# PaiDii/TGTC-Style

Hardware: AMD Instinct MI355X
Metric: rays/sec (128c+64f samples) on fern 400x400 (higher is better)
Workload: dtype f16 MFMA product + two block-scaled fp6 (e2m3) correction products, f32 accumulate (fine pass; coarse pass: fp16x3); 1 GPU; fern-shaped 400x400 frame, plain NeRF render (style off), 128 coarse + 64 fine samples/ray, one whole frame per rank per step, seeded random-init weights; precision=fp16x3+fp16mx

## Files before the change

tgtc-style_amd/csrc/mlp_nerf_fp16s.hip:

```cpp
#define TGTC_ASM_DMA 1
#include "mlp_nerf_mx.h"

#include <cstdlib>

#include "mlp_layouts.h"

namespace tgtc {

#ifndef TGTC_FP16S_INC
#define TGTC_FP16S_INC "fp16s_asm_nerf.inc"
#endif
#include TGTC_FP16S_INC

using CfgFp16s = MlpCfg<4, kFp16sTiles, false, 4>;
#ifndef TGTC_FRONT_ABL
#define TGTC_FRONT_ABL 0
#endif

__device__ __forceinline__ unsigned udiv_word(unsigned n) {
    unsigned z = (unsigned)(__builtin_amdgcn_rcpf((float)n) * 4294966784.0f);
    return z + __umulhi(z, (0u - n) * z);
}

template <int IN_MODE, int NCT>
__device__ __forceinline__ void fp16s_front(const NerfArgs& a, long long s_wave, half8 (&keep)[NCT][2], unsigned& bad) {
    const int lane = fresh_lane_id();
    const int g = lane >> 4, n = lane & 15;
    double pos[NCT][3], dir[NCT][3];
    long long sidx[NCT];
    half8 pe_h[2][NCT], pe_l[2][NCT], de_h[1][NCT], de_l[1][NCT];
    bad = 0;
#if TGTC_FRONT_ABL & 1
#pragma unroll
    for (int c = 0; c < NCT; ++c) pe_h[0][c] = pe_h[1][c] = half8{(_Float16)(float)(g + n)};
#else
    nerf_load_samples<NCT, IN_MODE>(a, s_wave, n, pos, dir, sidx);
    nerf_encode<NCT, false, false>(a, pos, dir, sidx, g, pe_h, pe_l, de_h, de_l);
#pragma unroll
    for (int c = 0; c < NCT; ++c)
        if (!(__builtin_fabs(pos[c][0]) <= kScreenBox && __builtin_fabs(pos[c][1]) <= kScreenBox && __builtin_fabs(pos[c][2]) <= kScreenBox))
            bad |= 1u << c;
#endif
#pragma unroll
    for (int c = 0; c < NCT; ++c) keep[c][0] = pe_h[0][c], keep[c][1] = pe_h[1][c];
}

template <int IN_MODE, bool FRONT>
__global__ void __launch_bounds__(256, 1) nerf_fp16s_kernel(NerfArgs a, long long n_pass) {
    using C = CfgFp16s;
    constexpr int NCT = C::NCT;
    using Ring = WeightStream<C, SingleStreamMap<NerfLayout::kFragsSigma>, true, true>;
    constexpr int kChunk = kFp16sChunkBytes, kSlots = C::RING_BYTES / kChunk, kLook = kSlots - 1, kPiece = kChunk / C::NWAVES;
    constexpr int kPad = ((NerfLayout::kFragsSigma * C::FRAG_BYTES + kChunk - 1) / kChunk + kSlots - 1) / kSlots * kSlots;
    static_assert(NerfLayout::kFragsSigma == kFp16sFrags && kPad == kFp16sPadChunks && C::RING_BYTES == 131072 && C::FRAG_BYTES == 1024 &&
                      kPiece % 4096 == 0 && kChunk == kChunkBytes,
                  "the generated stream was laid out for this ring");
    static_assert(kFp16sBox == kScreenBox, "the generated front end tests positions against the HIP front end's box");
    static_assert(!FRONT || IN_MODE == IN_RAYS, "the in-stream front end loads samples of rays");

    __shared__ __attribute__((aligned(16))) char smem[C::RING_BYTES + kNerfBiasBytes];
    const int wave = __builtin_amdgcn_readfirstlane(threadIdx.x >> 6);
    Ring ring;
    {
        const int lane = threadIdx.x & 63;
        const char* const streams[1] = {a.stream};
        ring.init(streams, smem, wave, lane);
#pragma unroll
        for (int j = 0; j < kNerfBiasBytes / (C::NWAVES * 1024); ++j)
            lds_dma16(a.bias + (j * C::NWAVES + wave) * 1024 + lane * 16, smem + C::RING_BYTES + (j * C::NWAVES + wave) * 1024);
        ring.lds_wave = smem + wave * kPiece;
        ring.voff = wave * kPiece + lane * 16;
        static_for<kLook * (kPiece / 1024)>([&](auto i_) {
            constexpr int i = decltype(i_)::value, ch = i / (kPiece / 1024), j = i % (kPiece / 1024);
            lds_dma16_s<(j % 4) * 1024>(ring.src[0] + ch * kChunk + (j / 4) * 4096, ring.voff, ring.lds_wave + ch * kChunk + (j / 4) * 4096);
        });
    }

    unsigned bad = 0;
    half8 keep[NCT][2];
    if constexpr (FRONT) {
        fp16s_front<IN_MODE>(a, (long long)blockIdx.x * C::SAMPLES_PER_WG + wave * C::SAMPLES_PER_WAVE, keep, bad);
        fp16s_asm_first_keep(keep);
    }
    const unsigned mm1 = (unsigned)(a.M - 1), zz = __builtin_amdgcn_readfirstlane(udiv_word((unsigned)a.N));

    for (long long p = blockIdx.x; p < n_pass; p += gridDim.x) {
        const long long s_wave = p * C::SAMPLES_PER_WG + wave * C::SAMPLES_PER_WAVE;
        if constexpr (!FRONT) fp16s_front<IN_MODE>(a, s_wave, keep, bad);
        const int fl = fresh_lane_id();
        ring.voff = wave * kPiece + fl * 16;
        ring.lane_lo = opaque((lds_cptr)smem + fl * 16);
        ring.lane_hi = opaque((lds_cptr)smem + 65536 + fl * 16);
        const lds_cptr bias_lane = opaque((lds_cptr)smem + C::RING_BYTES + 16 * (fl >> 4));
        float sigma[NCT];
        unsigned nbad = 0;
        if constexpr (FRONT) {
            const unsigned snext = (unsigned)(s_wave + (long long)gridDim.x * C::SAMPLES_PER_WG);
            fp16s_asm_nerf_sigma_pass_front(ring, bias_lane, sigma, nbad, a.ts, a.rays_o, a.rays_d, mm1, (unsigned)a.N, zz, snext);
        } else {
            fp16s_asm_nerf_sigma_pass(ring, bias_lane, keep, sigma);
        }
        const int lane = fresh_lane_id();
        if (lane < 16) {
#pragma unroll
            for (int c = 0; c < NCT; ++c) {
                const long long s = s_wave + c * 16 + lane;
                if (s < a.M) a.sigma[s] = (bad >> c & 1) ? __builtin_nanf("") : sigma[c];
            }
        }
        if constexpr (FRONT) bad = nbad;
    }
    wait_vmcnt<0>();
}

int nerf_fp16s_launch(const NerfArgs& a, hipStream_t st) {
    using C = CfgFp16s;
    if (a.M <= 0) return TGTC_OK;
    if (a.M >= 0x7fffffffLL) return fail(TGTC_ERR_UNSUPPORTED, "nerf: too many samples in one launch (%lld)", a.M);
    int cus = 0;
    if (const int rc = cu_count(cus)) return rc;
    const long long n_pass = (a.M + C::SAMPLES_PER_WG - 1) / C::SAMPLES_PER_WG;
    const unsigned grid = (unsigned)(n_pass < cus ? n_pass : cus);
    const char* e = std::getenv("TGTC_SCREEN_SERIAL_FRONT");
    if (e && e[0] == '1') nerf_fp16s_kernel<IN_RAYS, false><<<grid, C::NWAVES * 64, 0, st>>>(a, n_pass);
    else nerf_fp16s_kernel<IN_RAYS, true><<<grid, C::NWAVES * 64, 0, st>>>(a, n_pass);
    TGTC_LAUNCH_CHECK();
    return TGTC_OK;
}

}
```

tgtc-style_amd/csrc/mlp_nerf_front.h:

```cpp
#pragma once
#include "mlp_core.h"

namespace tgtc {

enum InMode { IN_RAYS = 0, IN_PTS = 1, IN_ENC = 2, IN_LIST = 3 };

struct NerfArgs {
    const char* bias;
    const char* stream;
    long long M;
    int N;
    const double* rays_o;
    const double* rays_d;
    const float* ts;
    const double* pts;
    const double* dirs;
    const float* pts_enc;
    const float* dirs_enc;
    float* rgb;
    float* sigma;
    float* remap;
    float* out_pts_enc;
    float* out_dirs_enc;
    const unsigned* live;
    const unsigned* n_live;
};

template <int NCT, int IN_MODE>
__device__ __forceinline__ void nerf_load_samples(const NerfArgs& a, long long s_wave, int n, double (&pos)[NCT][3],
                                                  double (&dir)[NCT][3], long long (&sidx)[NCT], unsigned n_live = 0) {
#pragma unroll
    for (int c = 0; c < NCT; ++c) {
        long long s = s_wave + c * 16 + n;
        if constexpr (IN_MODE == IN_LIST) {
            const unsigned i = (unsigned long long)s < n_live ? (unsigned)s : n_live - 1;
            s = a.live[i];
        }
        sidx[c] = s;
        if (s >= a.M) s = a.M - 1;
        if constexpr (IN_MODE == IN_RAYS || IN_MODE == IN_LIST) {
            const long long r = (unsigned)s / (unsigned)a.N;
            const double t = (double)a.ts[s];
#pragma unroll
            for (int k = 0; k < 3; ++k) {
                dir[c][k] = a.rays_d[r * 3 + k];
                pos[c][k] = a.rays_o[r * 3 + k] + t * dir[c][k];
            }
        } else if constexpr (IN_MODE == IN_PTS) {
#pragma unroll
            for (int k = 0; k < 3; ++k) pos[c][k] = a.pts[s * 3 + k], dir[c][k] = a.dirs[s * 3 + k];
        }
        if constexpr (IN_MODE != IN_ENC) {
#pragma unroll
            for (int k = 0; k < 3; ++k) asm volatile("" : "+v"(pos[c][k]), "+v"(dir[c][k]));
        }
    }
}

template <int NCT, bool SPLIT, bool FULL>
__device__ __forceinline__ void nerf_load_encoded(const NerfArgs& a, const long long (&sidx)[NCT], int g,
                                                  half8 (&pe_h)[2][NCT], half8 (&pe_l)[2][NCT], half8 (&de_h)[1][NCT],
                                                  half8 (&de_l)[1][NCT]) {
#pragma unroll
    for (int c = 0; c < NCT; ++c) {
        const long long s = sidx[c] < a.M ? sidx[c] : a.M - 1;
        half8 h2[2], l2[2];
        load_encoded_point<SPLIT>(a.pts_enc + s * 63, g, h2, l2);
        pe_h[0][c] = h2[0], pe_h[1][c] = h2[1], pe_l[0][c] = l2[0], pe_l[1][c] = l2[1];
        if constexpr (FULL) load_encoded_dir<SPLIT>(a.dirs_enc + s * 27, g, de_h[0][c], de_l[0][c]);
    }
}

template <int NCT, bool SPLIT, bool FULL>
__device__ __forceinline__ void nerf_encode(const NerfArgs& a, const double (&pos)[NCT][3], const double (&dir)[NCT][3],
                                            const long long (&sidx)[NCT], int g, half8 (&pe_h)[2][NCT],
                                            half8 (&pe_l)[2][NCT], half8 (&de_h)[1][NCT], half8 (&de_l)[1][NCT]) {
#pragma unroll
    for (int c = 0; c < NCT; ++c) {
        const bool live = sidx[c] < a.M;
        half8 h2[2], l2[2];
        encode_point<SPLIT, SPLIT>(pos[c], g, h2, l2, (a.out_pts_enc && live) ? a.out_pts_enc + sidx[c] * 63 : nullptr);
        pe_h[0][c] = h2[0], pe_h[1][c] = h2[1], pe_l[0][c] = l2[0], pe_l[1][c] = l2[1];
        if constexpr (FULL) {
            bool same = false;
            if constexpr (NCT > 1) {
                if (c > 0 && !a.out_dirs_enc)
                    same = __all(dir[c][0] == dir[c - 1][0] && dir[c][1] == dir[c - 1][1] && dir[c][2] == dir[c - 1][2]);
            }
            if (same) {
                de_h[0][c] = de_h[0][c > 0 ? c - 1 : 0], de_l[0][c] = de_l[0][c > 0 ? c - 1 : 0];
            } else {
                encode_dir<SPLIT, SPLIT>(dir[c], g, de_h[0][c], de_l[0][c],
                                         (a.out_dirs_enc && live) ? a.out_dirs_enc + sidx[c] * 27 : nullptr);
            }
        }
    }
}

template <int IN_MODE, bool SPLIT>
__device__ __forceinline__ void nerf_encode_dir_late(const NerfArgs& a, long long sidx, int g, half8& de_h, half8& de_l) {
    const long long s = sidx < a.M ? sidx : a.M - 1;
    if constexpr (IN_MODE == IN_ENC) {
        load_encoded_dir<SPLIT>(a.dirs_enc + s * 27, g, de_h, de_l);
    } else {
        double d[3];
        const double* src = (IN_MODE == IN_RAYS || IN_MODE == IN_LIST) ? a.rays_d + ((unsigned)s / (unsigned)a.N) * 3 : a.dirs + s * 3;
#pragma unroll
        for (int k = 0; k < 3; ++k) d[k] = src[k];
        encode_dir<SPLIT, SPLIT>(d, g, de_h, de_l, (a.out_dirs_enc && sidx < a.M) ? a.out_dirs_enc + sidx * 27 : nullptr);
    }
}

}
```

tgtc-style_amd/csrc/mlp_nerf_x3s.hip:

```cpp
#define TGTC_ASM_DMA 1
#include "mlp_nerf_mx.h"

#include "mlp_layouts.h"

namespace tgtc {

#ifndef TGTC_X3S_INC
#define TGTC_X3S_INC "x3_asm_nerf.inc"
#endif
#include TGTC_X3S_INC

using CfgX3s = MlpCfg<4, 2, true, 4>;
#ifndef TGTC_FRONT_ABL
#define TGTC_FRONT_ABL 0
#endif

template <int IN_MODE>
__global__ void __launch_bounds__(256, 1) nerf_x3s_kernel(NerfArgs a, long long n_pass) {
    using C = CfgX3s;
    unsigned n_live = 0;
    if constexpr (IN_MODE == IN_LIST) {
        n_live = __builtin_amdgcn_readfirstlane(*a.n_live);
        n_pass = ((long long)n_live + C::SAMPLES_PER_WG - 1) / C::SAMPLES_PER_WG;
    }
    using Ring = WeightStream<C, SingleStreamMap<NerfLayout::kFragsSigma>, true, true>;
    constexpr int kChunk = kX3sChunkBytes, kSlots = C::RING_BYTES / kChunk, kLook = kSlots - 1, kPiece = kChunk / C::NWAVES;
    constexpr int kPad = ((NerfLayout::kFragsSigma * C::FRAG_BYTES + kChunk - 1) / kChunk + kSlots - 1) / kSlots * kSlots;
    static_assert(NerfLayout::kFragsSigma == kX3sFrags && kPad == kX3sPadChunks && C::RING_BYTES == 131072 && C::FRAG_BYTES == 2048 && kPiece % 4096 == 0,
                  "the generated stream was laid out for this ring");

    __shared__ __attribute__((aligned(16))) char smem[C::RING_BYTES + kNerfBiasBytes];
    const int wave = __builtin_amdgcn_readfirstlane(threadIdx.x >> 6);
    Ring ring;
    {
        const int lane = threadIdx.x & 63;
        const char* const streams[1] = {a.stream};
        ring.init(streams, smem, wave, lane);
#pragma unroll
        for (int j = 0; j < kNerfBiasBytes / (C::NWAVES * 1024); ++j)
            lds_dma16(a.bias + (j * C::NWAVES + wave) * 1024 + lane * 16, smem + C::RING_BYTES + (j * C::NWAVES + wave) * 1024);
        ring.lds_wave = smem + wave * kPiece;
        ring.voff = wave * kPiece + lane * 16;
        static_for<kLook * (kPiece / 1024)>([&](auto i_) {
            constexpr int i = decltype(i_)::value, ch = i / (kPiece / 1024), j = i % (kPiece / 1024);
            lds_dma16_s<(j % 4) * 1024>(ring.src[0] + ch * kChunk + (j / 4) * 4096, ring.voff, ring.lds_wave + ch * kChunk + (j / 4) * 4096);
        });
    }

    for (long long p = blockIdx.x; p < n_pass; p += gridDim.x) {
        const long long s_wave = p * C::SAMPLES_PER_WG + wave * C::SAMPLES_PER_WAVE;
        half8 keep[2][4];
        {
            const int lane = fresh_lane_id();
            const int g = lane >> 4, n = lane & 15;
            double pos[2][3], dir[2][3];
            long long sidx[2];
            half8 pe_h[2][2], pe_l[2][2], de_h[1][2], de_l[1][2];
#if TGTC_FRONT_ABL & 1
#pragma unroll
            for (int c = 0; c < 2; ++c) pe_h[0][c] = pe_h[1][c] = pe_l[0][c] = pe_l[1][c] = half8{(_Float16)(float)(g + n)};
#elif TGTC_FRONT_ABL & 4
            nerf_load_samples<2, IN_RAYS>(a, s_wave, n, pos, dir, sidx);
#pragma unroll
            for (int c = 0; c < 2; ++c)
                pe_h[0][c] = pe_h[1][c] = pe_l[0][c] = pe_l[1][c] = half8{(_Float16)(float)(pos[c][0] + pos[c][1] + pos[c][2])};
#else
            if constexpr (IN_MODE == IN_LIST) nerf_load_samples<2, IN_LIST>(a, s_wave, n, pos, dir, sidx, n_live);
            else nerf_load_samples<2, IN_RAYS>(a, s_wave, n, pos, dir, sidx);
            nerf_encode<2, true, false>(a, pos, dir, sidx, g, pe_h, pe_l, de_h, de_l);
#endif
#pragma unroll
            for (int c = 0; c < 2; ++c) keep[c][0] = pe_h[0][c], keep[c][1] = pe_h[1][c], keep[c][2] = pe_l[0][c], keep[c][3] = pe_l[1][c];
        }
        const int fl = fresh_lane_id();
        ring.voff = wave * kPiece + fl * 16;
        ring.lane_lo = opaque((lds_cptr)smem + fl * 16);
        ring.lane_hi = opaque((lds_cptr)smem + 65536 + fl * 16);
        const lds_cptr bias_lane = opaque((lds_cptr)smem + C::RING_BYTES + 16 * (fl >> 4));
        float sigma[2];
        x3_asm_nerf_sigma_pass(ring, wave, bias_lane, keep, sigma);
        const int lane = fresh_lane_id();
        if (lane < 16) {
#pragma unroll
            for (int c = 0; c < 2; ++c) {
                if constexpr (IN_MODE == IN_LIST) {
                    const unsigned long long slot = (unsigned long long)(s_wave + c * 16 + lane);
                    if (slot < n_live) {
                        const unsigned s = a.live[slot];
                        if (s < a.M) a.sigma[s] = sigma[c];
                    }
                    continue;
                }
                const long long s = s_wave + c * 16 + lane;
                if (s < a.M) a.sigma[s] = sigma[c];
            }
        }
    }
    wait_vmcnt<0>();
}

int nerf_x3s_launch(const NerfArgs& a, hipStream_t st) {
    using C = CfgX3s;
    int cus = 0;
    if (const int rc = cu_count(cus)) return rc;
    const long long n_pass = (a.M + C::SAMPLES_PER_WG - 1) / C::SAMPLES_PER_WG;
    nerf_x3s_kernel<IN_RAYS><<<(unsigned)(n_pass < cus ? n_pass : cus), C::NWAVES * 64, 0, st>>>(a, n_pass);
    TGTC_LAUNCH_CHECK();
    return TGTC_OK;
}

int nerf_x3s_list_launch(const NerfArgs& a, hipStream_t st) {
    using C = CfgX3s;
    int cus = 0;
    if (const int rc = cu_count(cus)) return rc;
    const long long n_pass = (a.M + C::SAMPLES_PER_WG - 1) / C::SAMPLES_PER_WG;
    nerf_x3s_kernel<IN_LIST><<<(unsigned)(n_pass < cus ? n_pass : cus), C::NWAVES * 64, 0, st>>>(a, 0);
    TGTC_LAUNCH_CHECK();
    return TGTC_OK;
}

}
```

Measured before the change: 3.238 million rays/s.

## Overlap next pass's sample loading and encoding inside x3s sigma assembly stream

Moves the x3s (fp16x3) sigma kernel's per-pass front end, which loads ray samples and does the positional encoding, into the generated assembly sigma pass. That pass prefetches and encodes the next pass's samples (snext) while the current MLP runs, for both the ray and live-list modes. The aim is to hide the serial load and encode latency that used to run before each pass's MFMA work. In exchange it relies on a new generated include whose code is not shown, adds register pressure, and keeps an env-var fallback to the serial path.

After: 3.254 million rays/s, median of 6. No clear change (+0.5%).

```diff
diff --git a/tgtc-style_amd/csrc/mlp_nerf_fp16s.hip b/tgtc-style_amd/csrc/mlp_nerf_fp16s.hip
--- a/tgtc-style_amd/csrc/mlp_nerf_fp16s.hip
+++ b/tgtc-style_amd/csrc/mlp_nerf_fp16s.hip
@@ -16,11 +16,6 @@
 #ifndef TGTC_FRONT_ABL
 #define TGTC_FRONT_ABL 0
 #endif
-
-__device__ __forceinline__ unsigned udiv_word(unsigned n) {
-    unsigned z = (unsigned)(__builtin_amdgcn_rcpf((float)n) * 4294966784.0f);
-    return z + __umulhi(z, (0u - n) * z);
-}
 
 template <int IN_MODE, int NCT>
 __device__ __forceinline__ void fp16s_front(const NerfArgs& a, long long s_wave, half8 (&keep)[NCT][2], unsigned& bad) {
diff --git a/tgtc-style_amd/csrc/mlp_nerf_front.h b/tgtc-style_amd/csrc/mlp_nerf_front.h
--- a/tgtc-style_amd/csrc/mlp_nerf_front.h
+++ b/tgtc-style_amd/csrc/mlp_nerf_front.h
@@ -57,6 +57,11 @@
     }
 }
 
+__device__ __forceinline__ unsigned udiv_word(unsigned n) {
+    unsigned z = (unsigned)(__builtin_amdgcn_rcpf((float)n) * 4294966784.0f);
+    return z + __umulhi(z, (0u - n) * z);
+}
+
 template <int NCT, bool SPLIT, bool FULL>
 __device__ __forceinline__ void nerf_load_encoded(const NerfArgs& a, const long long (&sidx)[NCT], int g,
                                                   half8 (&pe_h)[2][NCT], half8 (&pe_l)[2][NCT], half8 (&de_h)[1][NCT],
diff --git a/tgtc-style_amd/csrc/mlp_nerf_x3s.hip b/tgtc-style_amd/csrc/mlp_nerf_x3s.hip
--- a/tgtc-style_amd/csrc/mlp_nerf_x3s.hip
+++ b/tgtc-style_amd/csrc/mlp_nerf_x3s.hip
@@ -1,5 +1,7 @@
 #define TGTC_ASM_DMA 1
 #include "mlp_nerf_mx.h"
+
+#include <cstdlib>
 
 #include "mlp_layouts.h"
 
@@ -15,7 +17,32 @@
 #define TGTC_FRONT_ABL 0
 #endif
 
+#include "x3_front_asm_nerf.inc"
+
 template <int IN_MODE>
+__device__ __forceinline__ void x3s_front(const NerfArgs& a, long long s_wave, unsigned n_live, half8 (&keep)[2][4], long long (&sidx)[2]) {
+    const int lane = fresh_lane_id();
+    const int g = lane >> 4, n = lane & 15;
+    double pos[2][3], dir[2][3];
+    half8 pe_h[2][2], pe_l[2][2], de_h[1][2], de_l[1][2];
+#if TGTC_FRONT_ABL & 1
+#pragma unroll
+    for (int c = 0; c < 2; ++c) pe_h[0][c] = pe_h[1][c] = pe_l[0][c] = pe_l[1][c] = half8{(_Float16)(float)(g + n)}, sidx[c] = a.M;
+#elif TGTC_FRONT_ABL & 4
+    nerf_load_samples<2, IN_RAYS>(a, s_wave, n, pos, dir, sidx);
+#pragma unroll
+    for (int c = 0; c < 2; ++c)
+        pe_h[0][c] = pe_h[1][c] = pe_l[0][c] = pe_l[1][c] = half8{(_Float16)(float)(pos[c][0] + pos[c][1] + pos[c][2])};
+#else
+    if constexpr (IN_MODE == IN_LIST) nerf_load_samples<2, IN_LIST>(a, s_wave, n, pos, dir, sidx, n_live);
+    else nerf_load_samples<2, IN_RAYS>(a, s_wave, n, pos, dir, sidx);
+    nerf_encode<2, true, false>(a, pos, dir, sidx, g, pe_h, pe_l, de_h, de_l);
+#endif
+#pragma unroll
+    for (int c = 0; c < 2; ++c) keep[c][0] = pe_h[0][c], keep[c][1] = pe_h[1][c], keep[c][2] = pe_l[0][c], keep[c][3] = pe_l[1][c];
+}
+
+template <int IN_MODE, bool FRONT>
 __global__ void __launch_bounds__(256, 1) nerf_x3s_kernel(NerfArgs a, long long n_pass) {
     using C = CfgX3s;
     unsigned n_live = 0;
@@ -47,38 +74,35 @@
         });
     }
 
+    half8 keep[2][4];
+    long long sidx[2] = {0, 0};
+    if constexpr (FRONT) {
+        if ((long long)blockIdx.x < n_pass) {
+            x3s_front<IN_MODE>(a, (long long)blockIdx.x * C::SAMPLES_PER_WG + wave * C::SAMPLES_PER_WAVE, n_live, keep, sidx);
+            x3_asm_first_keep(keep);
+        }
+    }
+    const unsigned mm1 = (unsigned)(a.M - 1), zz = __builtin_amdgcn_readfirstlane(udiv_word((unsigned)a.N));
+
     for (long long p = blockIdx.x; p < n_pass; p += gridDim.x) {
         const long long s_wave = p * C::SAMPLES_PER_WG + wave * C::SAMPLES_PER_WAVE;
-        half8 keep[2][4];
-        {
-            const int lane = fresh_lane_id();
-            const int g = lane >> 4, n = lane & 15;
-            double pos[2][3], dir[2][3];
-            long long sidx[2];
-            half8 pe_h[2][2], pe_l[2][2], de_h[1][2], de_l[1][2];
-#if TGTC_FRONT_ABL & 1
-#pragma unroll
-            for (int c = 0; c < 2; ++c) pe_h[0][c] = pe_h[1][c] = pe_l[0][c] = pe_l[1][c] = half8{(_Float16)(float)(g + n)};
-#elif TGTC_FRONT_ABL & 4
-            nerf_load_samples<2, IN_RAYS>(a, s_wave, n, pos, dir, sidx);
-#pragma unroll
-            for (int c = 0; c < 2; ++c)
-                pe_h[0][c] = pe_h[1][c] = pe_l[0][c] = pe_l[1][c] = half8{(_Float16)(float)(pos[c][0] + pos[c][1] + pos[c][2])};
-#else
-            if constexpr (IN_MODE == IN_LIST) nerf_load_samples<2, IN_LIST>(a, s_wave, n, pos, dir, sidx, n_live);
-            else nerf_load_samples<2, IN_RAYS>(a, s_wave, n, pos, dir, sidx);
-            nerf_encode<2, true, false>(a, pos, dir, sidx, g, pe_h, pe_l, de_h, de_l);
-#endif
-#pragma unroll
-            for (int c = 0; c < 2; ++c) keep[c][0] = pe_h[0][c], keep[c][1] = pe_h[1][c], keep[c][2] = pe_l[0][c], keep[c][3] = pe_l[1][c];
-        }
+        if constexpr (!FRONT) x3s_front<IN_MODE>(a, s_wave, n_live, keep, sidx);
         const int fl = fresh_lane_id();
         ring.voff = wave * kPiece + fl * 16;
         ring.lane_lo = opaque((lds_cptr)smem + fl * 16);
         ring.lane_hi = opaque((lds_cptr)smem + 65536 + fl * 16);
         const lds_cptr bias_lane = opaque((lds_cptr)smem + C::RING_BYTES + 16 * (fl >> 4));
         float sigma[2];
-        x3_asm_nerf_sigma_pass(ring, wave, bias_lane, keep, sigma);
+        unsigned nidx[2] = {0, 0};
+        if constexpr (FRONT) {
+            const unsigned snext = (unsigned)(s_wave + (long long)gridDim.x * C::SAMPLES_PER_WG);
+            if constexpr (IN_MODE == IN_LIST)
+                x3_asm_nerf_sigma_pass_front_list(ring, wave, bias_lane, sigma, nidx, a.ts, a.rays_o, a.rays_d, mm1, (unsigned)a.N, zz, snext, a.live, n_live - 1);
+            else
+                x3_asm_nerf_sigma_pass_front_rays(ring, wave, bias_lane, sigma, a.ts, a.rays_o, a.rays_d, mm1, (unsigned)a.N, zz, snext);
+        } else {
+            x3_asm_nerf_sigma_pass(ring, wave, bias_lane, keep, sigma);
+        }
         const int lane = fresh_lane_id();
         if (lane < 16) {
 #pragma unroll
@@ -86,7 +110,9 @@
                 if constexpr (IN_MODE == IN_LIST) {
                     const unsigned long long slot = (unsigned long long)(s_wave + c * 16 + lane);
                     if (slot < n_live) {
-                        const unsigned s = a.live[slot];
+                        unsigned s;
+                        if constexpr (FRONT) s = (unsigned)sidx[c];
+                        else s = a.live[slot];
                         if (s < a.M) a.sigma[s] = sigma[c];
                     }
                     continue;
@@ -95,8 +121,14 @@
                 if (s < a.M) a.sigma[s] = sigma[c];
             }
         }
+        if constexpr (FRONT && IN_MODE == IN_LIST) sidx[0] = nidx[0], sidx[1] = nidx[1];
     }
     wait_vmcnt<0>();
+}
+
+static bool x3s_serial_front() {
+    const char* e = std::getenv("TGTC_X3S_SERIAL_FRONT");
+    return e && e[0] == '1';
 }
 
 int nerf_x3s_launch(const NerfArgs& a, hipStream_t st) {
@@ -104,7 +136,9 @@
     int cus = 0;
     if (const int rc = cu_count(cus)) return rc;
     const long long n_pass = (a.M + C::SAMPLES_PER_WG - 1) / C::SAMPLES_PER_WG;
-    nerf_x3s_kernel<IN_RAYS><<<(unsigned)(n_pass < cus ? n_pass : cus), C::NWAVES * 64, 0, st>>>(a, n_pass);
+    const unsigned grid = (unsigned)(n_pass < cus ? n_pass : cus);
+    if (x3s_serial_front()) nerf_x3s_kernel<IN_RAYS, false><<<grid, C::NWAVES * 64, 0, st>>>(a, n_pass);
+    else nerf_x3s_kernel<IN_RAYS, true><<<grid, C::NWAVES * 64, 0, st>>>(a, n_pass);
     TGTC_LAUNCH_CHECK();
     return TGTC_OK;
 }
@@ -114,7 +148,9 @@
     int cus = 0;
     if (const int rc = cu_count(cus)) return rc;
     const long long n_pass = (a.M + C::SAMPLES_PER_WG - 1) / C::SAMPLES_PER_WG;
-    nerf_x3s_kernel<IN_LIST><<<(unsigned)(n_pass < cus ? n_pass : cus), C::NWAVES * 64, 0, st>>>(a, 0);
+    const unsigned grid = (unsigned)(n_pass < cus ? n_pass : cus);
+    if (x3s_serial_front()) nerf_x3s_kernel<IN_LIST, false><<<grid, C::NWAVES * 64, 0, st>>>(a, 0);
+    else nerf_x3s_kernel<IN_LIST, true><<<grid, C::NWAVES * 64, 0, st>>>(a, 0);
     TGTC_LAUNCH_CHECK();
     return TGTC_OK;
 }
```
